# Yoshiki172/Deep-Learning-based-RGBA-Image-Compression-with-Masked-Window-based-Attention

Measured on NVIDIA B200. Metric: 768x512 RGBA images/s (AutoEncoderRGB_Journal encode + decode forward); masked-attn kernel % of roofline, higher is better.
Workload: dtype f32 (attention: fp16 hi+lo split operands, 3 tcgen05 passes, f32 accumulate = f32-faithful; 4x4 attention plain f32; GDN contraction bf16x3 split + f32 accumulate; convolutions fp16 hi+lo split operands, 3 tcgen05 passes, chunked f32 accumulation outside the tensor core = f32-faithful)

## Files before the change

### deep-learning-based-rgba-image-compression-with-masked-window-based-attention_b200/_abi.py

```python
from __future__ import annotations

import ctypes
import os
from ctypes import c_char_p, c_float, c_int, c_int32, c_int64, c_void_p, POINTER

import torch

_PKG_DIR = os.path.dirname(os.path.abspath(__file__))
LIB_PATH = os.path.join(_PKG_DIR, "libmwa_b200.so")

MWA_OK = 0
ALGO_AUTO, ALGO_SIMT, ALGO_TCGEN05 = 0, 1, 2
ABI_VERSION = 1

_SIGNATURES = {
    "mwa_b200_abi_version": (c_int, []),
    "mwa_b200_status_string": (c_char_p, [c_int]),
    "mwa_b200_last_cuda_error": (c_char_p, []),
    "gdn_param_bytes": (c_int64, [c_int]),
    "gdn_prepare": (c_int, [c_void_p, c_void_p, c_int, c_float, c_float, c_float, c_void_p, c_int64, c_void_p]),
    "gdn_forward": (c_int, [c_void_p, c_void_p, c_void_p, c_int64, c_int, c_int64, c_int, c_int, c_int, c_void_p]),
    "gdn_forward_planes": (c_int, [c_void_p, c_void_p, c_void_p, c_int, c_int, c_void_p, c_int64, c_int, c_int, c_int, c_int,
                                   c_void_p]),
    "gdn_backward_workspace_bytes": (c_int64, [c_int64, c_int, c_int64]),
    "gdn_backward": (c_int, [c_void_p, c_void_p, c_void_p, c_void_p, c_void_p, c_float, c_float, c_void_p, c_void_p,
                             c_void_p, c_void_p, c_int64, c_int64, c_int, c_int64, c_int, c_int, c_void_p]),
    "gdn_param_offset": (c_int64, [c_int, c_int]),
    "gdn_bwd_square": (c_int, [c_void_p, c_void_p, c_int64, c_void_p]),
    "gdn_bwd_dn": (c_int, [c_void_p, c_void_p, c_void_p, c_void_p, c_void_p, c_int64, c_int, c_int64, c_int, c_int,
                           c_void_p]),
    "gdn_bwd_dx": (c_int, [c_void_p, c_void_p, c_void_p, c_void_p, c_int64, c_void_p]),
    "gdn_bwd_finalize": (c_int, [c_void_p, c_void_p, c_void_p, c_void_p, c_float, c_float, c_void_p, c_void_p,
                                 c_void_p, c_int64, c_int, c_int64, c_int, c_void_p]),
    "mwa_param_bytes": (c_int64, [c_int, c_int, c_int]),
    "mwa_prepare": (c_int, [c_void_p, c_void_p, c_void_p, c_void_p, c_void_p, c_int, c_int, c_int, c_float,
                            c_void_p, c_int64, c_void_p]),
    "mwa_debug_set_timing_buffer": (None, [c_void_p]),
    "mwa_workspace_bytes": (c_int64, [c_int, c_int, c_int, c_int]),
    "mwa_fast_path_needs_nchw": (c_int, [c_int, c_int, c_int]),
    "conv_image_bytes": (c_int64, [c_int, c_int, c_int, c_int, c_int]),
    "conv_split_bytes": (c_int64, [c_int, c_int, c_int, c_int]),
    "conv_prepare": (c_int, [c_void_p, c_int, c_int, c_int, c_int, c_int, c_void_p, c_int64, c_void_p]),
    "conv_forward": (c_int, [c_void_p, c_int64, c_void_p, c_void_p, c_void_p, c_int64, c_void_p, c_void_p, c_void_p, c_int,
                             c_int, c_int, c_int, c_int, c_int, c_int, c_int, c_int, c_void_p]),
    "gemm_tokens_forward": (c_int, [c_void_p, c_int64, c_int, c_void_p, c_void_p, c_int, c_void_p, c_void_p, c_void_p, c_void_p,
                                    c_void_p]),
    "conv_act_split": (c_int, [c_void_p, c_int64, c_int, c_int, c_int, c_int, c_int, c_void_p, c_void_p, c_int, c_int, c_void_p]),
    "conv_forward_ex": (c_int, [c_void_p, c_int64, c_void_p, c_void_p, c_int, c_void_p, c_void_p, c_void_p, c_int64,
                                c_void_p, c_int64, c_void_p, c_int64, c_void_p, c_void_p, c_int, c_int, c_int, c_void_p,
                                c_int, c_int, c_int, c_int, c_int, c_int, c_int, c_int, c_int, c_void_p, c_void_p]),
    "mwa_forward": (c_int, [c_void_p, c_void_p, c_void_p, c_void_p, c_int, c_int, c_int, c_int, c_int, c_int, c_int,
                            c_int, c_int, c_void_p, c_void_p, c_int64, c_void_p]),
# ... 115 lines not shown
```

### deep-learning-based-rgba-image-compression-with-masked-window-based-attention_b200/csrc/common.cuh

```cuda
#pragma once
#include <cuda_fp16.h>
#include <cuda_runtime.h>
#include <stdint.h>

namespace b200 {

constexpr int kNumSMs = 148;

__device__ __forceinline__ uint32_t smem_u32(const void* p) {
    return static_cast<uint32_t>(__cvta_generic_to_shared(p));
}

__device__ __forceinline__ bool elect_one() {
    uint32_t pred;
    asm volatile(
        "{\n\t.reg .pred p;\n\t"
        "elect.sync _|p, 0xffffffff;\n\t"
        "selp.u32 %0, 1, 0, p;\n\t}\n"
        : "=r"(pred));
    return pred != 0;
}

__device__ __forceinline__ void mbar_init(uint64_t* bar, uint32_t count) {
    asm volatile("mbarrier.init.shared::cta.b64 [%0], %1;" ::"r"(smem_u32(bar)), "r"(count) : "memory");
// ... 32 lines not shown
}
__device__ __forceinline__ void mbar_wait(uint64_t* bar, uint32_t parity) {
    while (!mbar_try_wait(bar, parity)) {
    }
}

__device__ __forceinline__ void fence_proxy_async_smem() {
    asm volatile("fence.proxy.async.shared::cta;" ::: "memory");
}

__device__ __forceinline__ void bulk_g2s(void* dst_smem, const void* src_gmem, uint32_t bytes, uint64_t* bar) {
    asm volatile(
        "cp.async.bulk.shared::cluster.global.mbarrier::complete_tx::bytes [%0], [%1], %2, [%3];" ::"r"(
            smem_u32(dst_smem)),
        "l"(src_gmem), "r"(bytes), "r"(smem_u32(bar))
        : "memory");
}

template <uint32_t kCols>
__device__ __forceinline__ void tmem_alloc(uint32_t* dst_smem) {
    static_assert(kCols == 32 || kCols == 64 || kCols == 128 || kCols == 256 || kCols == 512, "pow2 >= 32");
    asm volatile("tcgen05.alloc.cta_group::1.sync.aligned.shared::cta.b32 [%0], %1;" ::"r"(smem_u32(dst_smem)),
                 "n"(kCols)
                 : "memory");
    asm volatile("tcgen05.relinquish_alloc_permit.cta_group::1.sync.aligned;" ::: "memory");
}
template <uint32_t kCols>
__device__ __forceinline__ void tmem_dealloc(uint32_t taddr) {
    asm volatile("tcgen05.dealloc.cta_group::1.sync.aligned.b32 %0, %1;" ::"r"(taddr), "n"(kCols) : "memory");
}
// ... 125 lines not shown
}
__device__ __forceinline__ void umma_f16_ts_lanes(uint32_t tmem_d, uint32_t tmem_a, uint64_t bdesc, uint32_t idesc,
                                                  uint32_t accumulate, uint32_t m0, uint32_t m1, uint32_t m2, uint32_t m3) {
    asm volatile(
        "{\n\t.reg .pred p;\n\t"
        "setp.ne.b32 p, %4, 0;\n\t"
        "tcgen05.mma.cta_group::1.kind::f16 [%0], [%1], %2, %3, {%5, %6, %7, %8}, p;\n\t}\n" ::"r"(tmem_d),
        "r"(tmem_a), "l"(bdesc), "r"(idesc), "r"(accumulate), "r"(m0), "r"(m1), "r"(m2), "r"(m3)
        : "memory");
}
constexpr uint32_t kUmmaBMajorMN = 1u << 16;
__device__ __forceinline__ void umma_commit(uint64_t* bar) {
    asm volatile("tcgen05.commit.cta_group::1.mbarrier::arrive::one.shared::cluster.b64 [%0];" ::"r"(smem_u32(bar))
                 : "memory");
}

__device__ __forceinline__ uint32_t cluster_ctarank() {
    uint32_t r;
    asm volatile("mov.u32 %0, %%cluster_ctarank;" : "=r"(r));
    return r;
}
__device__ __forceinline__ void cluster_sync_all() {
    asm volatile("barrier.cluster.arrive.release.aligned;" ::: "memory");
    asm volatile("barrier.cluster.wait.acquire.aligned;" ::: "memory");
}
__device__ __forceinline__ uint32_t cluster_map_shared(uint32_t local_smem_addr, uint32_t rank) {
    uint32_t r;
    asm volatile("mapa.shared::cluster.u32 %0, %1, %2;" : "=r"(r) : "r"(local_smem_addr), "r"(rank));
    return r;
}
// ... 75 lines not shown
```

### deep-learning-based-rgba-image-compression-with-masked-window-based-attention_b200/csrc/conv_tc.cu

```cuda
#include <cstring>
#include <cuda.h>
#include "common.cuh"
#include "params.cuh"
#include "status.cuh"

namespace b200 {
namespace {

__host__ __device__ constexpr int conv_colparts(int nbmax) { return nbmax <= 64 ? 2 : 4; }
__host__ __device__ constexpr int conv_threads(int nbmax) { return (3 + 4 * conv_colparts(nbmax)) * 32; }
constexpr int kMaxTaps = 25, kMaxClasses = 4, kMaxGroups = 4;
constexpr int kTileH = 16, kTileW = 8;
enum { kActNone = 0, kActGelu = 1, kActRelu = 2, kActQuant = 3, kActLrp = 4, kActGate = 5, kActAdd2 = 6 };

struct ConvIo {
    const float* bias;
    const float* residual;
    float* out;
    int64_t out_bs;
    const float* aux;
    int64_t aux_bs;
    float* out2;
    int64_t out2_bs;
    uint16_t* sp_hi;
// ... 25 lines not shown
    int hy, hx, oy0, ox0;
    int a_half;
    int act;
    int merged;
    int nslabs;
    int sa, sb;
    int bparts;
    int resident;
    int dual;
    int nbuf_log2, bstride;
    int ncat;
    int b_region;
    int chunk;
    int nchunks[kMaxClasses];
    int tiles_y, tiles_x;
};

__device__ __forceinline__ uint64_t umma_desc_k_sw128_sbo(uint32_t smem_addr, uint32_t sbo_bytes) {
    uint64_t d = 0;
    d |= static_cast<uint64_t>((smem_addr & 0x3FFFFu) >> 4);
    d |= static_cast<uint64_t>(1) << 16;
    d |= static_cast<uint64_t>(sbo_bytes >> 4) << 32;
    d |= static_cast<uint64_t>(1) << 46;
    d |= static_cast<uint64_t>(2) << 61;
    return d;
}

__device__ __forceinline__ void tma_load_5d(void* dst_smem, const void* map, int c0, int c1, int c2, int c3, int c4, uint64_t* bar) {
    asm volatile(
        "cp.async.bulk.tensor.5d.shared::cluster.global.tile.mbarrier::complete_tx::bytes [%0], [%1, {%2,%3,%4,%5,%6}], [%7];" ::"r"(
// ... 267 lines not shown
    uint64_t* part_full = bars + 24;
    uint64_t* part_empty = bars + 28;
    const uint32_t nbl = uint32_t(P.nbuf_log2), nbm = (1u << nbl) - 1u, bstride = uint32_t(P.bstride);
    const uint32_t b_bytes = uint32_t(P.nb) * 128u;
    const uint32_t b_entry = P.bparts == 2 ? b_bytes : 2u * b_bytes;
    const uint32_t a_slot = 2u * uint32_t(P.a_half);
    const uint32_t b_base = uint32_t(SA) * a_slot;
    if (threadIdx.x == 0) {
        if (sb & 1023u) __trap();
        for (int i = 0; i < SA; ++i) {
            mbar_init(a_full + i, 1);
            mbar_init(a_empty + i, 1);
        }
        for (int i = 0; i < SB; ++i) {
            mbar_init(b_full + i, 1);
            mbar_init(b_empty + i, 1);
        }
        for (int i = 0; i < 4; ++i) {
            mbar_init(part_full + i, 1);
            mbar_init(part_empty + i, 4 * conv_colparts(NBMAX) * 32);
        }
        fence_mbar_init();
    }
    if (warp == 1) tmem_alloc<512>(&tmem_slot);
    float* s_scale = reinterpret_cast<float*>(smem + b_base + P.b_region);
    float* s_bias = s_scale + P.Npad;
    for (int i = threadIdx.x; i < P.Npad; i += conv_threads(NBMAX)) {
        s_scale[i] = inv_scale[i] * (io.in_scale ? 1.f / __ldg(io.in_scale) : 1.f);
        const int co = P.merged ? (i & 7) : i;
        s_bias[i] = (io.bias != nullptr && co < P.Cout) ? io.bias[co] : 0.f;
    }
    for (int i = threadIdx.x; i < kMaxClasses * kMaxTaps; i += conv_threads(NBMAX)) {
        const ConvTap tp = P.taps[i / kMaxTaps][i % kMaxTaps];
        s_tap[i] = make_uint2(uint32_t(tp.row) * 8u, uint32_t(tp.slab * P.KB * 2) * ((uint32_t(P.nb) * 128u) >> 4));
    }
    tc_fence_before_sync();
    __syncthreads();
    tc_fence_after_sync();
    const uint32_t tm = tmem_slot;

    const int tiles_img = P.tiles_y * P.tiles_x;
    const int ntiles = P.B * tiles_img * P.ncls * P.nblocks;
    struct TileIt {
        int nblk, tx, ty, cls, b;
        int d_nblk, d_tx, d_ty, d_cls, d_b;
        __device__ __forceinline__ void init(int t, int step, const ConvPlan& P) {
            auto split = [&](int v, int& nb_, int& tx_, int& ty_, int& cl_, int& b_) {
                nb_ = v % P.nblocks; v /= P.nblocks;
                tx_ = v % P.tiles_x; v /= P.tiles_x;
                ty_ = v % P.tiles_y; v /= P.tiles_y;
                cl_ = v % P.ncls;
                b_ = v / P.ncls;
            };
            split(t, nblk, tx, ty, cls, b);
            split(step, d_nblk, d_tx, d_ty, d_cls, d_b);
        }
        __device__ __forceinline__ void next(const ConvPlan& P) {
            nblk += d_nblk; int carry = nblk >= P.nblocks; nblk -= carry ? P.nblocks : 0;
            tx += d_tx + carry; carry = tx >= P.tiles_x; tx -= carry ? P.tiles_x : 0;
            ty += d_ty + carry; carry = ty >= P.tiles_y; ty -= carry ? P.tiles_y : 0;
            cls += d_cls + carry; carry = cls >= P.ncls; cls -= carry ? P.ncls : 0;
            b += d_b + carry;
        }
    };
    const int64_t slab_bytes = int64_t(P.KB) * 2 * P.Npad * 128;
    TileIt it;
    it.init(blockIdx.x, gridDim.x, P);

    auto dual_issue = [&](int p) {
        const uint32_t idesc = umma_idesc(kFmtF16, kFmtF16, 128, uint32_t(P.nb));
        const uint32_t idesc2 = umma_idesc(kFmtF16, kFmtF16, 128, 2u * uint32_t(P.nb));
        const uint64_t desc_c = (uint64_t(1) << 16) | (uint64_t(1) << 46) | (uint64_t(2) << 61);
        const uint64_t a_desc_c = desc_c | (uint64_t(((P.tw == 8 ? uint32_t(P.hx) : 8u) * 128u) >> 4) << 32);
        const uint64_t b_desc_c = desc_c | (uint64_t(1024 >> 4) << 32);
        const uint32_t b_addr16 = (sb + b_base) >> 4, b16 = b_bytes >> 4, a_half16 = uint32_t(P.a_half) >> 4;
        const int ntap = P.ntaps[0];
        const bool cat = NBMAX <= 64 && P.ncat;
        const int ksteps = (min(64, P.Cin) + 15) >> 4;
        const uint32_t d = tm + uint32_t(p) * 256;
        mbar_wait(b_full, 0);
        tc_fence_after_sync();
        for (int j = p; blockIdx.x + int64_t(j) * gridDim.x < ntiles; j += 2) {
// ... 21 lines not shown
                        umma_f16_ss(d, a_hi + ks * 2, b_hi + ks * 2, idesc, (tap | ks) ? 1u : 0u);
                        umma_f16_ss(d, a_lo + ks * 2, b_hi + ks * 2, idesc, 1u);
                        umma_f16_ss(d, a_hi + ks * 2, b_lo + ks * 2, idesc, 1u);
                    }
                }
            }
            umma_commit(a_empty + sa);
            umma_commit(part_full + p);
        }
    };

    if (warp == 0) {
        if (elect_one()) {
            uint32_t s = 0, ph = 0, first = 1;
            const uint32_t box_bytes = uint32_t(P.hy * P.hx) * 128u;
            for (int t = blockIdx.x; t < ntiles; t += gridDim.x, it.next(P)) {
                const int nblk = it.nblk, cls = it.cls, b = it.b, ty = it.ty, tx = it.tx;
                for (int g = 0; g < P.ngroups[cls]; ++g) {
                    const int plane = P.groups[cls][g].plane;
                    for (int kb = 0; kb < P.KB; ++kb) {
                        if (!first) mbar_wait(a_empty + s, ph ^ 1);
                        uint8_t* st = smem + s * a_slot;
                        mbar_arrive_expect_tx(a_full + s, 2u * box_bytes);
                        tma_load_5d(st, &map_hi, kb * 64, tx * P.tw + P.ox0, ty * P.th + P.oy0, plane, b, a_full + s);
                        tma_load_5d(st + P.a_half, &map_lo, kb * 64, tx * P.tw + P.ox0, ty * P.th + P.oy0, plane, b, a_full + s);
                        if (++s == uint32_t(SA)) { s = 0; ph ^= 1; first = 0; }
                    }
                }
            }
        }
    } else if (warp == 2 + 4 * conv_colparts(NBMAX)) {
        if (elect_one()) {
            if (P.resident) {
                mbar_arrive_expect_tx(b_full, uint32_t(P.b_region));
                for (uint32_t o = 0; o < uint32_t(P.b_region); o += 32768u)
                    bulk_g2s(smem + b_base + o, image + o, min(32768u, uint32_t(P.b_region) - o), b_full);
                if (P.dual) dual_issue(1);
            } else {
                uint32_t s = 0, ph = 0, first = 1;
                for (int t = blockIdx.x; t < ntiles; t += gridDim.x, it.next(P)) {
                    const int nblk = it.nblk, cls = it.cls, b = it.b, ty = it.ty, tx = it.tx;
                    for (int g = 0; g < P.ngroups[cls]; ++g) {
                        const ConvGroup gr = P.groups[cls][g];
                        for (int kb = 0; kb < P.KB; ++kb) {
                            for (int tap = gr.first; tap < gr.first + gr.ntaps; ++tap) {
                                const uint8_t* wsrc = image + P.taps[cls][tap].slab * slab_bytes + int64_t(kb) * 2 * P.Npad * 128 +
                                                      int64_t(nblk) * b_bytes;
                                if (P.bparts == 1) {
                                    if (!first) mbar_wait(b_empty + s, ph ^ 1);
                                    mbar_arrive_expect_tx(b_full + s, 2u * b_bytes);
                                    bulk_g2s(smem + b_base + s * b_entry, wsrc, b_bytes, b_full + s);
                                    bulk_g2s(smem + b_base + s * b_entry + b_bytes, wsrc + int64_t(P.Npad) * 128, b_bytes, b_full + s);
                                    if (++s == uint32_t(SB)) { s = 0; ph ^= 1; first = 0; }
                                } else {
#pragma unroll 1
                                    for (int part = 0; part < 2; ++part) {
                                        if (!first) mbar_wait(b_empty + s, ph ^ 1);
                                        mbar_arrive_expect_tx(b_full + s, b_bytes);
                                        bulk_g2s(smem + b_base + s * b_entry, wsrc + int64_t(part) * P.Npad * 128, b_bytes, b_full + s);
                                        if (++s == uint32_t(SB)) { s = 0; ph ^= 1; first = 0; }
                                    }
                                }
                            }
                        }
                    }
                }
            }
        }
    } else if (warp == 1) {
        if (P.dual) {
            if (elect_one()) dual_issue(0);
        } else if (elect_one()) {
            const uint32_t idesc = umma_idesc(kFmtF16, kFmtF16, 128, uint32_t(P.nb));
            const uint32_t idesc2 = umma_idesc(kFmtF16, kFmtF16, 128, 2u * uint32_t(P.nb));
            const bool cat = NBMAX <= 64 && P.ncat;
            const uint64_t desc_c = (uint64_t(1) << 16) | (uint64_t(1) << 46) | (uint64_t(2) << 61);
            const uint64_t a_desc_c = desc_c | (uint64_t(((P.tw == 8 ? uint32_t(P.hx) : 8u) * 128u) >> 4) << 32);
            const uint64_t b_desc_c = desc_c | (uint64_t(1024 >> 4) << 32);
            const uint32_t b_addr16 = (sb + b_base) >> 4, b16 = b_bytes >> 4, be16 = b_entry >> 4, a_half16 = uint32_t(P.a_half) >> 4;
            uint32_t sa = 0, pha = 0, sq = 0, phb = 0, c = 0;
            if (P.resident) {
                mbar_wait(b_full, 0);
                tc_fence_after_sync();
            }
            for (int t = blockIdx.x; t < ntiles; t += gridDim.x, it.next(P)) {
                const int nblk = it.nblk, cls = it.cls, b = it.b, ty = it.ty, tx = it.tx;
                const int nunits = P.ntaps[cls] * P.KB;
                int i = 0, ic = 0;
                for (int g = 0; g < P.ngroups[cls]; ++g) {
                    const ConvGroup gr = P.groups[cls][g];
                    for (int kb = 0; kb < P.KB; ++kb) {
                        mbar_wait(a_full + sa, pha);
                        tc_fence_after_sync();
                        const uint32_t a_base16 = (sb + sa * a_slot) >> 4;
                        const int valid = min(64, P.Cin - kb * 64);
                        const int ksteps = (valid + 15) >> 4;
                        uint2 tq_next = s_tap[cls * kMaxTaps + gr.first];
                        for (int tap = gr.first; tap < gr.first + gr.ntaps; ++tap, ++i) {
                            const uint2 tq = tq_next;
                            tq_next = s_tap[cls * kMaxTaps + tap + 1];
                            const uint32_t buf = c & nbm;
                            if (ic == 0 && c > nbm) {
// ... 12 lines not shown
                                    baddr = b_addr16 + sq * be16;
                                }
                                const uint64_t b_hi = b_desc_c | uint64_t(baddr), b_lo = b_hi + b16;
                                if (cat) {
                                    for (int ks = 0; ks < ksteps; ++ks) {
                                        umma_f16_ss(d, a_hi + ks * 2, b_hi + ks * 2, idesc2, (ic | ks) ? 1u : 0u);
                                        umma_f16_ss(d, a_lo + ks * 2, b_hi + ks * 2, idesc, 1u);
                                    }
                                } else {
                                    for (int ks = 0; ks < ksteps; ++ks) {
                                        umma_f16_ss(d, a_hi + ks * 2, b_hi + ks * 2, idesc, (ic | ks) ? 1u : 0u);
                                        umma_f16_ss(d, a_lo + ks * 2, b_hi + ks * 2, idesc, 1u);
                                        umma_f16_ss(d, a_hi + ks * 2, b_lo + ks * 2, idesc, 1u);
                                    }
                                }
                                if (!P.resident) {
                                    umma_commit(b_empty + sq);
                                    if (++sq == uint32_t(SB)) { sq = 0; phb ^= 1; }
                                }
                            } else {
                                mbar_wait(b_full + sq, phb);
                                tc_fence_after_sync();
                                uint64_t bd = b_desc_c | uint64_t(b_addr16 + sq * be16);
                                for (int ks = 0; ks < ksteps; ++ks) {
                                    umma_f16_ss(d, a_hi + ks * 2, bd + ks * 2, idesc, (ic | ks) ? 1u : 0u);
                                    umma_f16_ss(d, a_lo + ks * 2, bd + ks * 2, idesc, 1u);
                                }
                                umma_commit(b_empty + sq);
                                if (++sq == uint32_t(SB)) { sq = 0; phb ^= 1; }
                                mbar_wait(b_full + sq, phb);
                                tc_fence_after_sync();
                                bd = b_desc_c | uint64_t(b_addr16 + sq * be16);
                                for (int ks = 0; ks < ksteps; ++ks) umma_f16_ss(d, a_hi + ks * 2, bd + ks * 2, idesc, 1u);
                                umma_commit(b_empty + sq);
                                if (++sq == uint32_t(SB)) { sq = 0; phb ^= 1; }
                            }
                            if (++ic == P.chunk || i == nunits - 1) {
                                umma_commit(part_full + buf);
                                ++c;
                                ic = 0;
                            }
                        }
                        umma_commit(a_empty + sa);
                        if (++sa == uint32_t(SA)) { sa = 0; pha ^= 1; }
                    }
                }
            }
        }
    } else {
        constexpr int NCQ = conv_colparts(NBMAX);
        constexpr int NBQ = (NBMAX / 8 + NCQ - 1) / NCQ * 8;
        const int q = warp & 3, cq = (warp - 2) >> 2;
        const int r = q * 32 + lane, ry = r >> P.tw_log2, rx = r & (P.tw - 1);
        const uint32_t lane_addr = static_cast<uint32_t>(q * 32) << 16;
        const int64_t ohw = int64_t(P.Ho) * P.Wo;
        const int gran = P.nb >> 3;
        const int col0 = (gran * cq / NCQ) * 8, ncols = (gran * (cq + 1) / NCQ) * 8 - col0;
        uint32_t c = 0;
        for (int t = blockIdx.x; t < ntiles; t += gridDim.x, it.next(P)) {
            const int nblk = it.nblk, cls = it.cls, b = it.b, ty = it.ty, tx = it.tx;
            const int m = ty * P.th + ry, nn = tx * P.tw + rx;
            const int oy = m * P.os + P.qy[cls], ox = nn * P.os + P.qx[cls];
            const bool inb = m < P.GH && nn < P.GW && oy < P.Ho && ox < P.Wo;
            const int64_t pix = int64_t(oy) * P.Wo + ox;
            const int cbase = nblk * P.nb + col0;
            const float* res = io.residual ? io.residual + (int64_t(b) * P.Cout + cbase) * ohw + pix : nullptr;
            const float* aux = io.aux ? io.aux + b * io.aux_bs + cbase * ohw + pix : nullptr;
            if (inb && (rx & 7) == 0 && P.os == 1) {
                if (res != nullptr)
                    for (int j = 0; j < ncols && cbase + j < P.Cout; ++j) asm volatile("prefetch.global.L2 [%0];" ::"l"(res + j * ohw));
                if (aux != nullptr)
                    for (int j = 0; j < ncols && cbase + j < P.Cout; ++j) asm volatile("prefetch.global.L2 [%0];" ::"l"(aux + j * ohw));
            }
            const int nchunks = kSingle ? 1 : P.nchunks[cls];
            uint32_t buf = 0;
// ... 105 lines not shown
                        case kActGelu: CONV_EPI(kActGelu); break;
                        case kActRelu: CONV_EPI(kActRelu); break;
                        case kActQuant: CONV_EPI(kActQuant); break;
                        case kActLrp: CONV_EPI(kActLrp); break;
                        case kActGate: CONV_EPI(kActGate); break;
                        case kActAdd2: CONV_EPI(kActAdd2); break;
                        default: CONV_EPI(kActNone); break;
                    }
#undef CONV_EPI
                }
            }
            tc_fence_before_sync();
            mbar_arrive(part_empty + buf);
        }
    }
    tc_fence_before_sync();
    __syncthreads();
    if (warp == 1) tmem_dealloc<512>(tm);
}

typedef CUresult (*EncodeTiledFn)(CUtensorMap*, CUtensorMapDataType, cuuint32_t, void*, const cuuint64_t*, const cuuint64_t*,
                                  const cuuint32_t*, const cuuint32_t*, CUtensorMapInterleave, CUtensorMapSwizzle,
                                  CUtensorMapL2promotion, CUtensorMapFloatOOBfill);

int conv_plane_map(const void* base, int B, int planes, int GH, int GW, int C, int Cpad, int box_w, int box_h, CUtensorMap* map) {
    static EncodeTiledFn encode = nullptr;
    if (encode == nullptr) {
        void* fn = nullptr;
        cudaDriverEntryPointQueryResult qres;
        MWA_TRY_CUDA(cudaGetDriverEntryPoint("cuTensorMapEncodeTiled", &fn, cudaEnableDefault, &qres), "conv_forward(tensor map)");
        if (fn == nullptr || qres != cudaDriverEntryPointSuccess) return MWA_ERR_UNSUPPORTED;
        encode = reinterpret_cast<EncodeTiledFn>(fn);
// ... 95 lines not shown
        int n = 0;
        for (int pl = 0; pl < nplanes; ++pl) {
            ConvGroup g;
            g.plane = int8_t(pl); g.first = int16_t(n); g.ntaps = 0;
            for (int t = 0; t < P.ntaps[c]; ++t)
                if (raw[c][t].plane == pl) {
                    P.taps[c][n].row = int16_t((raw[c][t].dy - dy0) * P.hx + (raw[c][t].dx - dx0));
                    P.taps[c][n].slab = int16_t(raw[c][t].slab);
                    ++n; ++g.ntaps;
                }
            if (g.ntaps > 0) P.groups[c][P.ngroups[c]++] = g;
        }
    }
    P.tiles_y = (P.GH + P.th - 1) / P.th;
    P.tiles_x = (P.GW + P.tw - 1) / P.tw;
    const int ksteps_full = ((Cin < 64 ? Cin : 64) + 15) / 16;
    int max_units = 0;
    for (int c = 0; c < P.ncls; ++c) max_units = P.ntaps[c] * P.KB > max_units ? P.ntaps[c] * P.KB : max_units;
    P.chunk = 36 / (3 * ksteps_full);
    if (P.chunk < 1) P.chunk = 1;
    if (max_units * 3 * ksteps_full <= 64) P.chunk = max_units;
    for (int c = 0; c < P.ncls; ++c) P.nchunks[c] = (P.ntaps[c] * P.KB + P.chunk - 1) / P.chunk;
    P.sa = 2;
    const int budget = 200 * 1024 - 2 * P.Npad * 4 - P.sa * 2 * P.a_half;
    const int64_t image = int64_t(P.nslabs) * P.KB * 2 * P.Npad * 128;
    P.bparts = P.nb > 96 ? 2 : 1;
    if (P.nblocks == 1 && image <= budget) {
        P.resident = 1; P.bparts = 1; P.sb = 1; P.b_region = int(image);
    } else {
        const int entry = P.nb * 128 * (P.bparts == 2 ? 1 : 2);
// ... 4 lines not shown
    }
    P.dual = P.resident && P.ncls == 1 && P.ngroups[0] == 1 && P.KB == 1 && P.nchunks[0] == 1 && P.ntaps[0] > 1;
    P.ncat = P.nb <= 64 ? 1 : 0;
    P.nbuf_log2 = (P.nb <= 128 && !P.dual) ? 2 : 1;
    P.bstride = P.nbuf_log2 == 2 ? 128 : 256;
    if (P.dual) {
        const int room = 224 * 1024 - 2 * P.Npad * 4 - P.b_region;
        P.sa = room / (2 * P.a_half);
        if (P.sa > 4) P.sa = 4;
        if (P.sa < 2) P.sa = 2;
    }
    return MWA_OK;
}

int conv_smem_bytes(const ConvPlan& P) { return P.sa * 2 * P.a_half + P.b_region + 2 * P.Npad * 4 + 1024; }

}
}

using namespace b200;

extern "C" {

int64_t conv_image_bytes(int kind, int Cin, int Cout, int k, int stride) {
    ConvPlan P;
    if (Cin <= 0 || Cout <= 0 || build_plan(P, kind, 1, Cin, Cout, 16, 16, k, stride, 0) != MWA_OK) return MWA_ERR_UNSUPPORTED;
    return int64_t(P.nslabs) * P.KB * 2 * P.Npad * 128 + int64_t(P.Npad) * 4;
}

int64_t conv_split_bytes(int B, int Cin, int H, int W) {
// ... 70 lines not shown
    if (out_hi != nullptr) {
        if (!aligned16(out_hi) || !aligned16(out_lo)) return MWA_ERR_ALIGNMENT;
        if ((out_ps != 1 && out_ps != 2) || out_cstride % 8 != 0 || out_coff % 8 != 0 || out_coff < 0 ||
            out_coff + (Cout + 7) / 8 * 8 > out_cstride || P.Ho % out_ps != 0 || P.Wo % out_ps != 0)
            return MWA_ERR_INVALID;
        io.sp_hi = static_cast<uint16_t*>(out_hi); io.sp_lo = static_cast<uint16_t*>(out_lo);
        io.sp_ps = out_ps; io.sp_cstride = out_cstride; io.sp_coff = out_coff; io.sp_cvalid = (Cout + 7) / 8 * 8;
    }
    CUtensorMap mh, ml;
    memset(&mh, 0, sizeof(mh));
    memset(&ml, 0, sizeof(ml));
    rc = conv_plane_map(in_hi, B, ps * ps, H / ps, W / ps, Cin, cstride, P.hx, P.hy, &mh);
    if (rc != MWA_OK) return rc;
    rc = conv_plane_map(in_lo, B, ps * ps, H / ps, W / ps, Cin, cstride, P.hx, P.hy, &ml);
    if (rc != MWA_OK) return rc;
    const int smem = conv_smem_bytes(P);
    const int ntiles = B * P.tiles_y * P.tiles_x * P.ncls * P.nblocks;
    const int grid = ntiles < kNumSMs ? ntiles : kNumSMs;
    const uint8_t* img = static_cast<const uint8_t*>(image);
    const float* inv_scale = reinterpret_cast<const float*>(img + int64_t(P.nslabs) * P.KB * 2 * P.Npad * 128);
#define CONV_LAUNCH_K(NB, SINGLE)                                                                                              \
    do {                                                                                                                       \
        MWA_TRY_CUDA(cudaFuncSetAttribute(conv_tc_kernel<NB, false, SINGLE>, cudaFuncAttributeMaxDynamicSharedMemorySize, smem), \
                     "conv_forward(attr)");                                                                                    \
        conv_tc_kernel<NB, false, SINGLE><<<grid, conv_threads(NB), smem, st>>>(mh, ml, img, inv_scale, io, P);                \
    } while (0)
#define CONV_LAUNCH(NB)                                                                                                        \
    do {                                                                                                                       \
        if (NB >= 128 && single) CONV_LAUNCH_K(NB, (NB >= 128));                                                               \
        else CONV_LAUNCH_K(NB, false);                                                                                         \
    } while (0)
    bool single = true;
    for (int c = 0; c < P.ncls; ++c) single = single && P.nchunks[c] == 1;
    if (out_cl) {
        MWA_TRY_CUDA(cudaFuncSetAttribute(conv_tc_kernel<192, true>, cudaFuncAttributeMaxDynamicSharedMemorySize, smem),
                     "gemm_tokens_forward(attr)");
        conv_tc_kernel<192, true><<<grid, conv_threads(192), smem, st>>>(mh, ml, img, inv_scale, io, P);
        return check_launch("gemm_tokens_forward");
    }
    if (P.nb <= 32) CONV_LAUNCH(32);
    else if (P.nb <= 64) CONV_LAUNCH(64);
    else if (P.nb <= 128) CONV_LAUNCH(128);
    else CONV_LAUNCH(192);
#undef CONV_LAUNCH
#undef CONV_LAUNCH_K
    return check_launch("conv_forward");
}

int conv_forward_ex(const float* x, int64_t x_batch_stride, void* in_hi, void* in_lo, int in_cstride,
                    const float* bias, const float* residual, float* out, int64_t out_batch_stride, const float* aux,
                    int64_t aux_batch_stride, float* out2, int64_t out2_batch_stride, void* out_hi, void* out_lo,
                    int out_ps, int out_cstride, int out_coff, const void* image, int kind, int B, int Cin, int Cout, int H,
                    int W, int k, int stride, int act, const float* in_scale, void* stream) {
    return conv_forward_impl(x, x_batch_stride, in_hi, in_lo, in_cstride, bias, residual, out, out_batch_stride, aux,
                             aux_batch_stride, out2, out2_batch_stride, out_hi, out_lo, out_ps, out_cstride, out_coff, image,
                             kind, B, Cin, Cout, H, W, k, stride, act, in_scale, stream, 0);
}

int gemm_tokens_forward(const float* x, int64_t T, int Cin, const float* bias, float* out, int Cout, const void* image,
                        void* split_hi, void* split_lo, const float* in_scale, void* stream) {
    if (!x || !out || !image || !split_hi || !split_lo || T < 0 || Cin <= 0 || Cout <= 0) return MWA_ERR_INVALID;
// ... 26 lines not shown
```

### include/mwa_b200.h

```cpp
#ifndef MWA_B200_H_
#define MWA_B200_H_

#include <stdint.h>

#if defined(__GNUC__)
#define MWA_API __attribute__((visibility("default")))
#else
#define MWA_API
#endif

#ifdef __cplusplus
extern "C" {
#endif

#define MWA_B200_ABI_VERSION 1

enum {
    MWA_OK = 0,
    MWA_ERR_INVALID = -1,
    MWA_ERR_UNSUPPORTED = -2,
    MWA_ERR_ALIGNMENT = -3,
    MWA_ERR_WORKSPACE = -4,
    MWA_ERR_CUDA = -5
};
// ... 21 lines not shown
MWA_API int gdn_bwd_square(const float* x, float* x2, int64_t n, void* stream);
MWA_API int gdn_bwd_dn(const float* grad_y, const float* x, float* n_to_term1, const void* params, float* dn,
                       int64_t n_img, int C, int64_t hw, int inverse, int channels_last, void* stream);
MWA_API int gdn_bwd_dx(const float* term1, const float* x, const float* t, float* grad_x, int64_t n, void* stream);
MWA_API int gdn_bwd_finalize(const float* dn, const float* dgamma_eff, const float* beta_p, const float* gamma_p,
                             float beta_bound, float gamma_bound, float* grad_beta_p, float* grad_gamma_p,
                             float* dbeta_scratch, int64_t n_img, int C, int64_t hw, int channels_last, void* stream);

MWA_API int64_t mwa_param_bytes(int C, int heads, int ws);
MWA_API int mwa_prepare(const float* qkv_w, const float* qkv_b, const float* proj_w, const float* proj_b,
                const float* bias_table, int C, int heads, int ws, float scale, void* params,
                int64_t params_bytes, void* stream);
MWA_API int64_t mwa_workspace_bytes(int B, int H, int W, int ws);
MWA_API int mwa_fast_path_needs_nchw(int C, int heads, int ws);
MWA_API void mwa_debug_set_timing_buffer(void* device_u64x8192);
MWA_API int mwa_forward(const float* x, const float* alpha, float* out, const void* params, int B, int C, int H, int W,
                int heads, int ws, int shift, int channels_last, int algo, int32_t* kept_count, void* workspace,
                int64_t workspace_bytes, void* stream);

MWA_API int window_attention_forward(const float* xw, const float* mask, float* out, const void* params, int64_t K,
                                     int C, int heads, int ws, int mask_windows, void* stream);

MWA_API int mwa_backward(const float* x, const float* alpha, const float* grad_out, const float* qkv_w,
                         const float* proj_w, const void* params, float* grad_x, float* grad_table, float* xw_tok,
                         float* ao_tok, float* dy_tok, float* dqkv_tok, int B, int C, int H, int W, int heads, int ws,
                         int shift, int channels_last, void* stream);
MWA_API int window_attention_backward(const float* xw, const float* mask, const float* grad_out, const float* qkv_w,
                                      const float* proj_w, const void* params, float* grad_xw, float* grad_table,
                                      float* ao_tok, float* dqkv_tok, int64_t K, int C, int heads, int ws,
                                      int mask_windows, void* stream);
// ... 82 lines not shown
```

Baseline: 387.6.

## Multicast conv weight slabs across 2-CTA clusters via TMA multicast

Conv tiles are regrouped so that CTAs in a cluster of two work on neighbouring spatial tiles with the same weight block. Each CTA loads one piece of the weight stage and multicasts it to the whole cluster. Releases use multicast tcgen05 commits, so one fetch of weight bytes from L2 serves both CTAs. The cost is cross-CTA barrier coupling, padding groups that may leave one CTA idle, cluster occupancy queries, and a tail drain before exit.

```diff
diff --git a/deep-learning-based-rgba-image-compression-with-masked-window-based-attention_b200/_abi.py b/deep-learning-based-rgba-image-compression-with-masked-window-based-attention_b200/_abi.py
--- a/deep-learning-based-rgba-image-compression-with-masked-window-based-attention_b200/_abi.py
+++ b/deep-learning-based-rgba-image-compression-with-masked-window-based-attention_b200/_abi.py
@@ -36,6 +36,7 @@
     "mwa_prepare": (c_int, [c_void_p, c_void_p, c_void_p, c_void_p, c_void_p, c_int, c_int, c_int, c_float,
                             c_void_p, c_int64, c_void_p]),
     "mwa_debug_set_timing_buffer": (None, [c_void_p]),
+    "conv_set_cluster_override": (c_int, [c_int]),
     "mwa_workspace_bytes": (c_int64, [c_int, c_int, c_int, c_int]),
     "mwa_fast_path_needs_nchw": (c_int, [c_int, c_int, c_int]),
     "conv_image_bytes": (c_int64, [c_int, c_int, c_int, c_int, c_int]),
diff --git a/deep-learning-based-rgba-image-compression-with-masked-window-based-attention_b200/csrc/common.cuh b/deep-learning-based-rgba-image-compression-with-masked-window-based-attention_b200/csrc/common.cuh
--- a/deep-learning-based-rgba-image-compression-with-masked-window-based-attention_b200/csrc/common.cuh
+++ b/deep-learning-based-rgba-image-compression-with-masked-window-based-attention_b200/csrc/common.cuh
@@ -70,6 +70,14 @@
         "cp.async.bulk.shared::cluster.global.mbarrier::complete_tx::bytes [%0], [%1], %2, [%3];" ::"r"(
             smem_u32(dst_smem)),
         "l"(src_gmem), "r"(bytes), "r"(smem_u32(bar))
+        : "memory");
+}
+__device__ __forceinline__ void bulk_g2s_multicast(void* dst_smem, const void* src_gmem, uint32_t bytes, uint64_t* bar,
+                                                   uint16_t cta_mask) {
+    asm volatile(
+        "cp.async.bulk.shared::cluster.global.mbarrier::complete_tx::bytes.multicast::cluster [%0], [%1], %2, [%3], %4;" ::"r"(
+            smem_u32(dst_smem)),
+        "l"(src_gmem), "r"(bytes), "r"(smem_u32(bar)), "h"(cta_mask)
         : "memory");
 }
 
@@ -225,6 +233,12 @@
     asm volatile("tcgen05.commit.cta_group::1.mbarrier::arrive::one.shared::cluster.b64 [%0];" ::"r"(smem_u32(bar))
                  : "memory");
 }
+__device__ __forceinline__ void umma_commit_multicast(uint64_t* bar, uint16_t cta_mask) {
+    asm volatile("tcgen05.commit.cta_group::1.mbarrier::arrive::one.shared::cluster.multicast::cluster.b64 [%0], %1;" ::"r"(
+                     smem_u32(bar)),
+                 "h"(cta_mask)
+                 : "memory");
+}
 
 __device__ __forceinline__ uint32_t cluster_ctarank() {
     uint32_t r;
diff --git a/deep-learning-based-rgba-image-compression-with-masked-window-based-attention_b200/csrc/conv_tc.cu b/deep-learning-based-rgba-image-compression-with-masked-window-based-attention_b200/csrc/conv_tc.cu
--- a/deep-learning-based-rgba-image-compression-with-masked-window-based-attention_b200/csrc/conv_tc.cu
+++ b/deep-learning-based-rgba-image-compression-with-masked-window-based-attention_b200/csrc/conv_tc.cu
@@ -1,4 +1,5 @@
 #include <cstring>
+#include <mutex>
 #include <cuda.h>
 #include "common.cuh"
 #include "params.cuh"
@@ -63,6 +64,8 @@
     int chunk;
     int nchunks[kMaxClasses];
     int tiles_y, tiles_x;
+    int cluster;
+    int pgroups;
 };
 
 __device__ __forceinline__ uint64_t umma_desc_k_sw128_sbo(uint32_t smem_addr, uint32_t sbo_bytes) {
@@ -360,7 +363,7 @@
         }
         for (int i = 0; i < SB; ++i) {
             mbar_init(b_full + i, 1);
-            mbar_init(b_empty + i, 1);
+            mbar_init(b_empty + i, P.cluster);
         }
         for (int i = 0; i < 4; ++i) {
             mbar_init(part_full + i, 1);
@@ -383,35 +386,48 @@
     tc_fence_before_sync();
     __syncthreads();
     tc_fence_after_sync();
+    if (P.cluster > 1) cluster_sync_all();
     const uint32_t tm = tmem_slot;
 
     const int tiles_img = P.tiles_y * P.tiles_x;
     const int ntiles = P.B * tiles_img * P.ncls * P.nblocks;
+    const uint32_t crank = blockIdx.x % uint32_t(P.cluster);
+    const int cid = blockIdx.x / P.cluster, nclusters = gridDim.x / P.cluster;
+    const int ngroups = P.B * P.pgroups * P.ncls * P.nblocks;
     struct TileIt {
-        int nblk, tx, ty, cls, b;
-        int d_nblk, d_tx, d_ty, d_cls, d_b;
-        __device__ __forceinline__ void init(int t, int step, const ConvPlan& P) {
-            auto split = [&](int v, int& nb_, int& tx_, int& ty_, int& cl_, int& b_) {
+        int nblk, pg, cls, b;
+        int d_nblk, d_pg, d_cls, d_b;
+        int tx, ty;
+        bool valid;
+        __device__ __forceinline__ void locate(const ConvPlan& P, int tiles_img, uint32_t rank) {
+            const int p = pg * P.cluster + int(rank);
+            valid = p < tiles_img;
+            ty = p / P.tiles_x;
+            tx = p - ty * P.tiles_x;
+        }
+        __device__ __forceinline__ void init(int t, int step, const ConvPlan& P, int tiles_img, uint32_t rank) {
+            auto split = [&](int v, int& nb_, int& pg_, int& cl_, int& b_) {
                 nb_ = v % P.nblocks; v /= P.nblocks;
-                tx_ = v % P.tiles_x; v /= P.tiles_x;
-                ty_ = v % P.tiles_y; v /= P.tiles_y;
+                pg_ = v % P.pgroups; v /= P.pgroups;
                 cl_ = v % P.ncls;
                 b_ = v / P.ncls;
             };
-            split(t, nblk, tx, ty, cls, b);
-            split(step, d_nblk, d_tx, d_ty, d_cls, d_b);
-        }
-        __device__ __forceinline__ void next(const ConvPlan& P) {
+            split(t, nblk, pg, cls, b);
+            split(step, d_nblk, d_pg, d_cls, d_b);
+            locate(P, tiles_img, rank);
+        }
+        __device__ __forceinline__ void next(const ConvPlan& P, int tiles_img, uint32_t rank) {
             nblk += d_nblk; int carry = nblk >= P.nblocks; nblk -= carry ? P.nblocks : 0;
-            tx += d_tx + carry; carry = tx >= P.tiles_x; tx -= carry ? P.tiles_x : 0;
-            ty += d_ty + carry; carry = ty >= P.tiles_y; ty -= carry ? P.tiles_y : 0;
+            pg += d_pg + carry; carry = pg >= P.pgroups; pg -= carry ? P.pgroups : 0;
             cls += d_cls + carry; carry = cls >= P.ncls; cls -= carry ? P.ncls : 0;
             b += d_b + carry;
+            locate(P, tiles_img, rank);
         }
     };
     const int64_t slab_bytes = int64_t(P.KB) * 2 * P.Npad * 128;
     TileIt it;
-    it.init(blockIdx.x, gridDim.x, P);
+    it.init(cid, nclusters, P, tiles_img, crank);
+#define CONV_FOR_GROUPS for (int t = cid; t < ngroups; t += nclusters, it.next(P, tiles_img, crank))
 
     auto dual_issue = [&](int p) {
         const uint32_t idesc = umma_idesc(kFmtF16, kFmtF16, 128, uint32_t(P.nb));
@@ -463,8 +479,9 @@
         if (elect_one()) {
             uint32_t s = 0, ph = 0, first = 1;
             const uint32_t box_bytes = uint32_t(P.hy * P.hx) * 128u;
-            for (int t = blockIdx.x; t < ntiles; t += gridDim.x, it.next(P)) {
-                const int nblk = it.nblk, cls = it.cls, b = it.b, ty = it.ty, tx = it.tx;
+            CONV_FOR_GROUPS {
+                const int cls = it.cls, b = it.b, ty = it.ty, tx = it.tx;
+                if (!it.valid) continue;
                 for (int g = 0; g < P.ngroups[cls]; ++g) {
                     const int plane = P.groups[cls][g].plane;
                     for (int kb = 0; kb < P.KB; ++kb) {
@@ -486,34 +503,46 @@
                     bulk_g2s(smem + b_base + o, image + o, min(32768u, uint32_t(P.b_region) - o), b_full);
                 if (P.dual) dual_issue(1);
             } else {
-                uint32_t s = 0, ph = 0, first = 1;
-                for (int t = blockIdx.x; t < ntiles; t += gridDim.x, it.next(P)) {
-                    const int nblk = it.nblk, cls = it.cls, b = it.b, ty = it.ty, tx = it.tx;
+                const uint32_t C = uint32_t(P.cluster), piece = b_bytes / C, poff = crank * piece;
+                const uint16_t cmask = uint16_t((1u << C) - 1u);
+                uint32_t s = 0, ph = 0, first = 1, produced = 0;
+                auto fill = [&](const uint8_t* src, uint32_t dst_off) {
+                    uint8_t* dst = smem + b_base + s * b_entry + dst_off;
+                    if (C == 1) bulk_g2s(dst, src, b_bytes, b_full + s);
+                    else bulk_g2s_multicast(dst + poff, src + poff, piece, b_full + s, cmask);
+                };
+                CONV_FOR_GROUPS {
+                    const int nblk = it.nblk, cls = it.cls;
                     for (int g = 0; g < P.ngroups[cls]; ++g) {
                         const ConvGroup gr = P.groups[cls][g];
                         for (int kb = 0; kb < P.KB; ++kb) {
                             for (int tap = gr.first; tap < gr.first + gr.ntaps; ++tap) {
                                 const uint8_t* wsrc = image + P.taps[cls][tap].slab * slab_bytes + int64_t(kb) * 2 * P.Npad * 128 +
                                                       int64_t(nblk) * b_bytes;
-                                if (P.bparts == 1) {
+#pragma unroll 1
+                                for (int part = 0; part < P.bparts; ++part) {
                                     if (!first) mbar_wait(b_empty + s, ph ^ 1);
-                                    mbar_arrive_expect_tx(b_full + s, 2u * b_bytes);
-                                    bulk_g2s(smem + b_base + s * b_entry, wsrc, b_bytes, b_full + s);
-                                    bulk_g2s(smem + b_base + s * b_entry + b_bytes, wsrc + int64_t(P.Npad) * 128, b_bytes, b_full + s);
+#if CONV_DIAG_WEIGHTS_ONCE
+                                    if (!first) {
+                                        mbar_arrive(b_full + s);
+                                        ++produced;
+                                        if (++s == uint32_t(SB)) { s = 0; ph ^= 1; first = 0; }
+                                        continue;
+                                    }
+#endif
+                                    mbar_arrive_expect_tx(b_full + s, b_entry);
+                                    fill(wsrc + int64_t(part) * P.Npad * 128, 0);
+                                    if (P.bparts == 1) fill(wsrc + int64_t(P.Npad) * 128, b_bytes);
+                                    ++produced;
                                     if (++s == uint32_t(SB)) { s = 0; ph ^= 1; first = 0; }
-                                } else {
-#pragma unroll 1
-                                    for (int part = 0; part < 2; ++part) {
-                                        if (!first) mbar_wait(b_empty + s, ph ^ 1);
-                                        mbar_arrive_expect_tx(b_full + s, b_bytes);
-                                        bulk_g2s(smem + b_base + s * b_entry, wsrc + int64_t(part) * P.Npad * 128, b_bytes, b_full + s);
-                                        if (++s == uint32_t(SB)) { s = 0; ph ^= 1; first = 0; }
-                                    }
                                 }
                             }
                         }
                     }
                 }
+                if (C > 1)
+                    for (uint32_t k = produced > uint32_t(SB) ? produced - uint32_t(SB) : 0u; k < produced; ++k)
+                        mbar_wait(b_empty + k % uint32_t(SB), (k / uint32_t(SB)) & 1u);
             }
         }
     } else if (warp == 1) {
@@ -528,13 +557,27 @@
             const uint64_t b_desc_c = desc_c | (uint64_t(1024 >> 4) << 32);
             const uint32_t b_addr16 = (sb + b_base) >> 4, b16 = b_bytes >> 4, be16 = b_entry >> 4, a_half16 = uint32_t(P.a_half) >> 4;
             uint32_t sa = 0, pha = 0, sq = 0, phb = 0, c = 0;
+            const uint16_t cmask = uint16_t((1u << P.cluster) - 1u);
+            auto release_b = [&]() {
+                if (P.cluster == 1) umma_commit(b_empty + sq);
+                else umma_commit_multicast(b_empty + sq, cmask);
+                if (++sq == uint32_t(SB)) { sq = 0; phb ^= 1; }
+            };
             if (P.resident) {
                 mbar_wait(b_full, 0);
                 tc_fence_after_sync();
             }
-            for (int t = blockIdx.x; t < ntiles; t += gridDim.x, it.next(P)) {
-                const int nblk = it.nblk, cls = it.cls, b = it.b, ty = it.ty, tx = it.tx;
+            CONV_FOR_GROUPS {
+                const int cls = it.cls;
                 const int nunits = P.ntaps[cls] * P.KB;
+                if (!it.valid) {
+                    for (int e = 0; e < nunits * P.bparts; ++e) {
+                        mbar_wait(b_full + sq, phb);
+                        for (uint32_t r = 0; r < uint32_t(P.cluster); ++r) mbar_arrive_cluster(cluster_map_shared(smem_u32(b_empty + sq), r));
+                        if (++sq == uint32_t(SB)) { sq = 0; phb ^= 1; }
+                    }
+                    continue;
+                }
                 int i = 0, ic = 0;
                 for (int g = 0; g < P.ngroups[cls]; ++g) {
                     const ConvGroup gr = P.groups[cls][g];
@@ -577,10 +620,7 @@
                                         umma_f16_ss(d, a_hi + ks * 2, b_lo + ks * 2, idesc, 1u);
                                     }
                                 }
-                                if (!P.resident) {
-                                    umma_commit(b_empty + sq);
-                                    if (++sq == uint32_t(SB)) { sq = 0; phb ^= 1; }
-                                }
+                                if (!P.resident) release_b();
                             } else {
                                 mbar_wait(b_full + sq, phb);
                                 tc_fence_after_sync();
@@ -589,14 +629,12 @@
                                     umma_f16_ss(d, a_hi + ks * 2, bd + ks * 2, idesc, (ic | ks) ? 1u : 0u);
                                     umma_f16_ss(d, a_lo + ks * 2, bd + ks * 2, idesc, 1u);
                                 }
-                                umma_commit(b_empty + sq);
-                                if (++sq == uint32_t(SB)) { sq = 0; phb ^= 1; }
+                                release_b();
                                 mbar_wait(b_full + sq, phb);
                                 tc_fence_after_sync();
                                 bd = b_desc_c | uint64_t(b_addr16 + sq * be16);
                                 for (int ks = 0; ks < ksteps; ++ks) umma_f16_ss(d, a_hi + ks * 2, bd + ks * 2, idesc, 1u);
-                                umma_commit(b_empty + sq);
-                                if (++sq == uint32_t(SB)) { sq = 0; phb ^= 1; }
+                                release_b();
                             }
                             if (++ic == P.chunk || i == nunits - 1) {
                                 umma_commit(part_full + buf);
@@ -620,8 +658,9 @@
         const int gran = P.nb >> 3;
         const int col0 = (gran * cq / NCQ) * 8, ncols = (gran * (cq + 1) / NCQ) * 8 - col0;
         uint32_t c = 0;
-        for (int t = blockIdx.x; t < ntiles; t += gridDim.x, it.next(P)) {
+        CONV_FOR_GROUPS {
             const int nblk = it.nblk, cls = it.cls, b = it.b, ty = it.ty, tx = it.tx;
+            if (!it.valid) continue;
             const int m = ty * P.th + ry, nn = tx * P.tw + rx;
             const int oy = m * P.os + P.qy[cls], ox = nn * P.os + P.qx[cls];
             const bool inb = m < P.GH && nn < P.GW && oy < P.Ho && ox < P.Wo;
@@ -757,8 +796,10 @@
             mbar_arrive(part_empty + buf);
         }
     }
+#undef CONV_FOR_GROUPS
     tc_fence_before_sync();
     __syncthreads();
+    if (P.cluster > 1) cluster_sync_all();
     if (warp == 1) tmem_dealloc<512>(tm);
 }
 
@@ -884,6 +925,8 @@
     }
     P.tiles_y = (P.GH + P.th - 1) / P.th;
     P.tiles_x = (P.GW + P.tw - 1) / P.tw;
+    P.cluster = 1;
+    P.pgroups = P.tiles_y * P.tiles_x;
     const int ksteps_full = ((Cin < 64 ? Cin : 64) + 15) / 16;
     int max_units = 0;
     for (int c = 0; c < P.ncls; ++c) max_units = P.ntaps[c] * P.KB > max_units ? P.ntaps[c] * P.KB : max_units;
@@ -918,6 +961,70 @@
 }
 
 int conv_smem_bytes(const ConvPlan& P) { return P.sa * 2 * P.a_half + P.b_region + 2 * P.Npad * 4 + 1024; }
+
+int g_cluster_override = 0;
+
+int pick_cluster(const ConvPlan& P) {
+    if (P.resident || P.dual) return 1;
+    if (g_cluster_override > 0) return g_cluster_override;
+    return 2;
+}
+
+void plan_set_cluster(ConvPlan& P, int C) {
+    P.cluster = C;
+    P.pgroups = (P.tiles_y * P.tiles_x + C - 1) / C;
+}
+
+int max_active_clusters(const void* kern, const cudaLaunchConfig_t& cfg, int C, int* out) {
+    struct Entry { const void* kern; int smem, C, n; };
+    static Entry cache[32];
+    static int ncache = 0;
+    static std::mutex mu;
+    std::lock_guard<std::mutex> lock(mu);
+    for (int i = 0; i < ncache; ++i)
+        if (cache[i].kern == kern && cache[i].smem == int(cfg.dynamicSmemBytes) && cache[i].C == C) {
+            *out = cache[i].n;
+            return MWA_OK;
+        }
+    int n = 0;
+    MWA_TRY_CUDA(cudaOccupancyMaxActiveClusters(&n, kern, &cfg), "conv_forward(cluster occupancy)");
+    if (n < 1) return MWA_ERR_UNSUPPORTED;
+    if (ncache < 32) cache[ncache++] = Entry{kern, int(cfg.dynamicSmemBytes), C, n};
+    *out = n;
+    return MWA_OK;
+}
+
+template <int NB, bool kCL, bool kSingle>
+int launch_conv(const CUtensorMap& mh, const CUtensorMap& ml, const uint8_t* img, const float* inv_scale, const ConvIo& io,
+                const ConvPlan& P, cudaStream_t st) {
+    auto kern = conv_tc_kernel<NB, kCL, kSingle>;
+    const int smem = conv_smem_bytes(P);
+    MWA_TRY_CUDA(cudaFuncSetAttribute(kern, cudaFuncAttributeMaxDynamicSharedMemorySize, smem), "conv_forward(attr)");
+    const int ngroups = P.B * P.pgroups * P.ncls * P.nblocks;
+    cudaLaunchConfig_t cfg;
+    memset(&cfg, 0, sizeof(cfg));
+    cudaLaunchAttribute attr[1];
+    cfg.blockDim = dim3(conv_threads(NB));
+    cfg.dynamicSmemBytes = size_t(smem);
+    cfg.stream = st;
+    int grid = ngroups < kNumSMs ? ngroups : kNumSMs;
+    if (P.cluster > 1) {
+        attr[0].id = cudaLaunchAttributeClusterDimension;
+        attr[0].val.clusterDim.x = unsigned(P.cluster);
+        attr[0].val.clusterDim.y = 1;
+        attr[0].val.clusterDim.z = 1;
+        cfg.attrs = attr;
+        cfg.numAttrs = 1;
+        cfg.gridDim = dim3(unsigned(kNumSMs / P.cluster * P.cluster));
+        int nclusters = 0;
+        const int rc = max_active_clusters(reinterpret_cast<const void*>(kern), cfg, P.cluster, &nclusters);
+        if (rc != MWA_OK) return rc;
+        grid = (ngroups < nclusters ? ngroups : nclusters) * P.cluster;
+    }
+    cfg.gridDim = dim3(unsigned(grid));
+    MWA_TRY_CUDA(cudaLaunchKernelEx(&cfg, kern, mh, ml, img, inv_scale, io, P), kCL ? "gemm_tokens_forward" : "conv_forward");
+    return check_launch(kCL ? "gemm_tokens_forward" : "conv_forward");
+}
 
 }
 }
@@ -1018,37 +1125,24 @@
     if (rc != MWA_OK) return rc;
     rc = conv_plane_map(in_lo, B, ps * ps, H / ps, W / ps, Cin, cstride, P.hx, P.hy, &ml);
     if (rc != MWA_OK) return rc;
-    const int smem = conv_smem_bytes(P);
-    const int ntiles = B * P.tiles_y * P.tiles_x * P.ncls * P.nblocks;
-    const int grid = ntiles < kNumSMs ? ntiles : kNumSMs;
+    plan_set_cluster(P, pick_cluster(P));
     const uint8_t* img = static_cast<const uint8_t*>(image);
     const float* inv_scale = reinterpret_cast<const float*>(img + int64_t(P.nslabs) * P.KB * 2 * P.Npad * 128);
-#define CONV_LAUNCH_K(NB, SINGLE)                                                                                              \
-    do {                                                                                                                       \
-        MWA_TRY_CUDA(cudaFuncSetAttribute(conv_tc_kernel<NB, false, SINGLE>, cudaFuncAttributeMaxDynamicSharedMemorySize, smem), \
-                     "conv_forward(attr)");                                                                                    \
-        conv_tc_kernel<NB, false, SINGLE><<<grid, conv_threads(NB), smem, st>>>(mh, ml, img, inv_scale, io, P);                \
-    } while (0)
-#define CONV_LAUNCH(NB)                                                                                                        \
-    do {                                                                                                                       \
-        if (NB >= 128 && single) CONV_LAUNCH_K(NB, (NB >= 128));                                                               \
-        else CONV_LAUNCH_K(NB, false);                                                                                         \
-    } while (0)
+    if (out_cl) return launch_conv<192, true, false>(mh, ml, img, inv_scale, io, P, st);
     bool single = true;
     for (int c = 0; c < P.ncls; ++c) single = single && P.nchunks[c] == 1;
-    if (out_cl) {
-        MWA_TRY_CUDA(cudaFuncSetAttribute(conv_tc_kernel<192, true>, cudaFuncAttributeMaxDynamicSharedMemorySize, smem),
-                     "gemm_tokens_forward(attr)");
-        conv_tc_kernel<192, true><<<grid, conv_threads(192), smem, st>>>(mh, ml, img, inv_scale, io, P);
-        return check_launch("gemm_tokens_forward");
-    }
-    if (P.nb <= 32) CONV_LAUNCH(32);
-    else if (P.nb <= 64) CONV_LAUNCH(64);
-    else if (P.nb <= 128) CONV_LAUNCH(128);
-    else CONV_LAUNCH(192);
-#undef CONV_LAUNCH
-#undef CONV_LAUNCH_K
-    return check_launch("conv_forward");
+    if (P.nb <= 32) return launch_conv<32, false, false>(mh, ml, img, inv_scale, io, P, st);
+    if (P.nb <= 64) return launch_conv<64, false, false>(mh, ml, img, inv_scale, io, P, st);
+    if (P.nb <= 128) return single ? launch_conv<128, false, true>(mh, ml, img, inv_scale, io, P, st)
+                                   : launch_conv<128, false, false>(mh, ml, img, inv_scale, io, P, st);
+    return single ? launch_conv<192, false, true>(mh, ml, img, inv_scale, io, P, st)
+                  : launch_conv<192, false, false>(mh, ml, img, inv_scale, io, P, st);
+}
+
+int conv_set_cluster_override(int cluster) {
+    if (cluster != 0 && cluster != 1 && cluster != 2 && cluster != 4) return MWA_ERR_INVALID;
+    g_cluster_override = cluster;
+    return MWA_OK;
 }
 
 int conv_forward_ex(const float* x, int64_t x_batch_stride, void* in_hi, void* in_lo, int in_cstride,
diff --git a/include/mwa_b200.h b/include/mwa_b200.h
--- a/include/mwa_b200.h
+++ b/include/mwa_b200.h
@@ -59,6 +59,7 @@
 MWA_API int64_t mwa_workspace_bytes(int B, int H, int W, int ws);
 MWA_API int mwa_fast_path_needs_nchw(int C, int heads, int ws);
 MWA_API void mwa_debug_set_timing_buffer(void* device_u64x8192);
+MWA_API int conv_set_cluster_override(int cluster);
 MWA_API int mwa_forward(const float* x, const float* alpha, float* out, const void* params, int B, int C, int H, int W,
                 int heads, int ws, int shift, int channels_last, int algo, int32_t* kept_count, void* workspace,
                 int64_t workspace_bytes, void* stream);
```

After: 386.0, median of 6. No clear change (-0.4%).
